# hallgeirl/cse168-raytracer

Measured on AMD Instinct MI355X. Metric: Mrays/s (primary+shadow), higher is better.
Workload: dtype f32; 1 GPU; sponza-standin 1920x1080 64spp primary+shadow; scene_triangles=76552, bvh_nodes=46701, math=exact: every quotient of the reference's slab and triangle tests, bit for bit, control_flow=while-while, ray_order=image order, resident_bytes_per_gpu=35765164

## Files before the change

### cse168-raytracer_amd/csrc/mr_api.cpp

```cpp
#include <algorithm>
#include <cmath>
#include <cstdarg>
#include <cstdio>
#include <cstring>
#include <new>
#include <vector>

#include "mr_internal.h"
#include "mr_tile.h"

namespace mr {

static thread_local char g_err[512] = "";

mr_status fail(mr_status code, const char *fmt, ...) {
    va_list ap;
    va_start(ap, fmt);
    vsnprintf(g_err, sizeof(g_err), fmt, ap);
    va_end(ap);
    return code;
}

namespace {

template <typename T>
mr_status upload(T *&dst, const T *src, size_t count, uint64_t &bytes) {
    const size_t sz = (count ? count : 1) * sizeof(T);
    MR_HIP_CHECK(hipMalloc(reinterpret_cast<void **>(&dst), sz));
    if (count) MR_HIP_CHECK(hipMemcpy(dst, src, count * sizeof(T), hipMemcpyHostToDevice));
    bytes += sz;
    return MR_OK;
}

void release_device(mr_scene *s) {
    DeviceScene &d = s->dev;
    (void)hipFree(d.nodes); (void)hipFree(d.tris); (void)hipFree(d.tri_prim); (void)hipFree(d.leaf_cnt_ext);
    (void)hipFree(d.v); (void)hipFree(d.n); (void)hipFree(d.vi); (void)hipFree(d.ni);
    (void)hipFree(d.materials); (void)hipFree(d.prim_material);
    (void)hipFree(d.spheres); (void)hipFree(d.planes);
    d = DeviceScene();
    (void)hipFree(s->d_stats); s->d_stats = nullptr;
    (void)hipFree(s->d_work_counters); s->d_work_counters = nullptr;
    for (EyeTables &t : s->eye_tables.set) {
        (void)hipFree(t.d);
        if (t.ready) (void)hipEventDestroy(static_cast<hipEvent_t>(t.ready));
        t = EyeTables();
    }
    s->eye_tables.calls = 0;
    (void)hipFree(s->d_stage_rays); (void)hipFree(s->d_stage_hits);
    s->d_stage_rays = s->d_stage_hits = nullptr;
    s->stage_cap = 0;
    for (void *e : s->stage_events) (void)hipEventDestroy(static_cast<hipEvent_t>(e));
    s->stage_events.clear();
    if (s->copy_in) (void)hipStreamDestroy(static_cast<hipStream_t>(s->copy_in));
    if (s->copy_out) (void)hipStreamDestroy(static_cast<hipStream_t>(s->copy_out));
    s->copy_in = s->copy_out = nullptr;
    (void)hipFree(s->d_occluded);
    s->d_occluded = nullptr;
    s->occluded_cap = 0;
    (void)hipFree(s->d_light_scale);
    s->d_light_scale = nullptr;
    s->light_scale_cap = 0;
}

inline int32_t leaf_ref(uint32_t first, uint32_t count) {
    const uint32_t c = count < (uint32_t)kLeafCountMask ? count : (uint32_t)kLeafCountMask;
    return (int32_t)~((first << kLeafCountBits) | c);
}

mr_status upload_materials(mr_scene *s);

std::vector<int32_t> node_storage_order(const HostTree &t, uint32_t mode) {
    std::vector<int32_t> order;
    const auto inner = [&](int32_t n) { return n >= 0 && !t.nodes[(size_t)n].is_leaf; };
    if (t.nodes.empty() || t.nodes[0].is_leaf) return order;
// ... 152 lines not shown
    if ((st = upload(d.tri_prim, rec_prim.data(), rec_prim.size(), d.bytes)) != MR_OK) return st;
    if ((st = upload(d.leaf_cnt_ext, cnt_ext.data(), cnt_ext.size(), d.bytes)) != MR_OK) return st;
    if ((st = upload(d.v, m.v.data(), m.v.size(), d.bytes)) != MR_OK) return st;
    if ((st = upload(d.n, m.n.data(), m.n.size(), d.bytes)) != MR_OK) return st;
    if ((st = upload(d.vi, m.vi.data(), m.vi.size(), d.bytes)) != MR_OK) return st;
    if ((st = upload(d.ni, m.ni.data(), m.ni.size(), d.bytes)) != MR_OK) return st;
    d.n_spheres = m.n_spheres();
    d.n_planes = m.n_planes();
    if (d.n_spheres) {
        std::vector<float4> sp(d.n_spheres);
        for (uint32_t i = 0; i < d.n_spheres; i++)
            sp[i] = make_float4(m.spheres[4 * i], m.spheres[4 * i + 1], m.spheres[4 * i + 2], m.spheres[4 * i + 3]);
        if ((st = upload(d.spheres, sp.data(), sp.size(), d.bytes)) != MR_OK) return st;
    }
    if (d.n_planes) {
        std::vector<float4> pl(2 * (size_t)d.n_planes);
        for (uint32_t i = 0; i < d.n_planes; i++) {
            float matf;
            memcpy(&matf, &m.plane_material[i], sizeof(matf));
            pl[2 * i] = make_float4(m.planes[6 * i], m.planes[6 * i + 1], m.planes[6 * i + 2], matf);
            pl[2 * i + 1] = make_float4(m.planes[6 * i + 3], m.planes[6 * i + 4], m.planes[6 * i + 5], 0.f);
        }
        if ((st = upload(d.planes, pl.data(), pl.size(), d.bytes)) != MR_OK) return st;
    }
    const HostNode &root = t.nodes[0];
    memcpy(d.root_lo, root.lo, sizeof(d.root_lo));
    memcpy(d.root_hi, root.hi, sizeof(d.root_hi));
    d.root_ref = ref_of(0);
    d.n_inner = n_inner;
    d.n_tris = n_rec;
    d.stack_depth = t.max_depth + 1;
    MR_HIP_CHECK(hipMalloc(reinterpret_cast<void **>(&s->d_stats), 2 * sizeof(unsigned long long)));
    MR_HIP_CHECK(hipMemset(s->d_stats, 0, 2 * sizeof(unsigned long long)));
    MR_HIP_CHECK(hipMalloc(reinterpret_cast<void **>(&s->d_work_counters), 2 * kWorkCounters * sizeof(unsigned long long)));
    MR_HIP_CHECK(hipMemset(s->d_work_counters, 0, 2 * kWorkCounters * sizeof(unsigned long long)));
    return upload_materials(s);
}

mr_status upload_materials(mr_scene *s) {
    DeviceScene &d = s->dev;
    if (!s->prim_material.empty() && s->prim_material.size() != s->mesh.n_triangles())
        return fail(MR_ERR_STATE, "mr_scene_set_materials covered %zu objects, the scene now holds %u: set the materials "
                                  "again after the last object was added", s->prim_material.size(), s->mesh.n_triangles());
    (void)hipFree(d.materials); (void)hipFree(d.prim_material);
    d.materials = nullptr; d.prim_material = nullptr;
    d.user_materials = s->materials.empty() ? 0u : 1u;
    d.refractive = 0;
    for (size_t i = 0; i + 10 < s->materials.size(); i += 11)
        if (s->materials[i + 6] > 0.f || s->materials[i + 7] > 0.f || s->materials[i + 8] > 0.f) d.refractive = 1;
    static const float white[11] = {1, 1, 1, 0, 0, 0, 0, 0, 0, 1, 1};
    const float *src = s->materials.empty() ? white : s->materials.data();
    const size_t nfl = s->materials.empty() ? 11 : s->materials.size();
    MR_HIP_CHECK(hipMalloc(reinterpret_cast<void **>(&d.materials), nfl * sizeof(float)));
    MR_HIP_CHECK(hipMemcpy(d.materials, src, nfl * sizeof(float), hipMemcpyHostToDevice));
    if (!s->prim_material.empty()) {
        MR_HIP_CHECK(hipMalloc(reinterpret_cast<void **>(&d.prim_material), s->prim_material.size() * sizeof(uint32_t)));
        MR_HIP_CHECK(hipMemcpy(d.prim_material, s->prim_material.data(), s->prim_material.size() * sizeof(uint32_t), hipMemcpyHostToDevice));
    }
    return MR_OK;
}

mr_status ensure_stage(mr_scene *s, uint64_t n) {
    if (n <= s->stage_cap) return MR_OK;
    (void)hipFree(s->d_stage_rays); (void)hipFree(s->d_stage_hits);
    s->d_stage_rays = s->d_stage_hits = nullptr;
    s->stage_cap = 0;
    MR_HIP_CHECK(hipMalloc(&s->d_stage_rays, n * sizeof(mr_ray)));
    MR_HIP_CHECK(hipMalloc(&s->d_stage_hits, n * sizeof(mr_hit)));
// ... 452 lines not shown
    for (uint32_t b = rank; b < nb; b += world) n += (b + 1) * band_rows <= H ? band_rows : H - b * band_rows;
    *rows = n;
    return MR_OK;
}

mr_status mr_deinterleave_bands(mr_scene *s, const float *d_recv, float *d_full, uint32_t W, uint32_t H, uint32_t band_rows,
                                uint32_t world, uint32_t shard_rows, uint32_t floats_per_pixel, void *stream) {
    mr_status st = require_device(s);
    if (st != MR_OK) return st;
    if (!d_recv || !d_full) return fail(MR_ERR_INVALID, "NULL argument");
    if (band_rows == 0 || world == 0 || floats_per_pixel == 0) return fail(MR_ERR_INVALID, "mr_deinterleave_bands: bad band description");
    for (uint32_t r = 0; r < world; r++) {
        uint32_t rows = 0;
        mr_band_rows_of(H, band_rows, r, world, &rows);
        if (rows > shard_rows) return fail(MR_ERR_INVALID, "rank %u owns %u rows, the shards hold %u", r, rows, shard_rows);
    }
    MR_HIP_CHECK(hipSetDevice(s->device));
    return launch_deinterleave(d_recv, d_full, W, H, band_rows, world, shard_rows, floats_per_pixel, static_cast<hipStream_t>(stream));
}

mr_status mr_render_direct(mr_scene *s, const mr_frame_desc *frame, float *d_rgb, mr_hit *d_hits, mr_hit *d_shadow_hits,
                           uint64_t *d_counts, void *stream) {
    mr_status st = require_device(s);
    if (st != MR_OK) return st;
    if (!frame || !d_rgb) return fail(MR_ERR_INVALID, "NULL argument");
    if (frame->W == 0 || frame->H == 0) return fail(MR_ERR_INVALID, "empty image");
    if ((reinterpret_cast<uintptr_t>(d_hits) & 15) || (reinterpret_cast<uintptr_t>(d_shadow_hits) & 15) ||
        (reinterpret_cast<uintptr_t>(d_counts) & 7) || (reinterpret_cast<uintptr_t>(d_rgb) & 3))
        return fail(MR_ERR_INVALID, "hit buffers must be 16-byte aligned, counters 8-byte aligned");
    mr_frame_desc fd = *frame;
    if (fd.band_world <= 1) { fd.band_world = 1; fd.band_rank = 0; if (fd.band_rows == 0) fd.band_rows = 1; }
    MR_HIP_CHECK(hipSetDevice(s->device));
    return launch_frame(s->dev, fd, d_rgb, d_hits, d_shadow_hits, reinterpret_cast<unsigned long long *>(d_counts),
                        s->d_work_counters + kWorkCounters + (s->next_counter.fetch_add(1) % kWorkCounters), s->eye_tables,
                        static_cast<hipStream_t>(stream));
}

mr_status mr_scene_set_materials(mr_scene *s, const mr_material *mats, uint32_t n_mats, const uint32_t *prim_material) {
    if (!s || !mats || n_mats == 0) return fail(MR_ERR_INVALID, "NULL argument or no materials");
    const uint32_t nt = s->mesh.n_triangles();
    if (prim_material)
        for (uint32_t i = 0; i < nt; i++)
            if (prim_material[i] >= n_mats) return fail(MR_ERR_INVALID, "triangle %u has material %u of %u", i, prim_material[i], n_mats);
    for (uint32_t i = 0; i < s->mesh.n_planes(); i++)
        if (s->mesh.plane_material[i] >= n_mats)
            return fail(MR_ERR_INVALID, "plane %u has material %u of %u", i, s->mesh.plane_material[i], n_mats);
    s->materials.resize(11 * (size_t)n_mats);
    for (uint32_t i = 0; i < n_mats; i++) {
        float *o = &s->materials[11 * (size_t)i];
        for (int c = 0; c < 3; c++) {
            const float ks = mats[i].specular[c];
            const float kt = fmaxf(fminf(mats[i].transmission[c], 1.0f - ks), 0.f);
            const float kd = fmaxf(fminf(mats[i].diffuse[c], 1.0f - ks - kt), 0.f);
            o[c] = kd; o[3 + c] = ks; o[6 + c] = kt;
        }
        o[9] = mats[i].shininess;
        o[10] = mats[i].refract_index;
    }
    if (prim_material) s->prim_material.assign(prim_material, prim_material + nt);
    else s->prim_material.clear();
    if (s->on_device) {
        MR_HIP_CHECK(hipSetDevice(s->device));
        MR_HIP_CHECK(hipDeviceSynchronize());
        return upload_materials(s);
    }
    return MR_OK;
}
// ... 161 lines not shown
```

### cse168-raytracer_amd/csrc/mr_frame.hip

```cpp
#include <hip/hip_runtime.h>

#include <cstring>

#include "mr_eye.h"
#include "mr_internal.h"
#include "mr_phong.h"
#include "mr_recursion.h"
#include "mr_surface.h"
#include "mr_tile.h"
#include "mr_traverse.h"

namespace mr {
namespace {

struct FrameArgs {
    EyeFrame eye;
    TraceParams tp;
    SurfacePtrs m;
    DirectLight lt;
    const float *mats;
    const uint32_t *prim_mat;
    mr_hit *hits;
    mr_hit *shadow_hits;
    float *rgb;
    unsigned long long *counts;
    uint32_t body_wgs, body_iters, tail_base, tail_chunks;
    unsigned *tail_counter;
    float4 *rel_nodes, *rel_tris;
    float rel_root_lo[3], rel_root_hi[3];
    uint32_t build, n_inner, n_rec;
};

__device__ __forceinline__ void eye_tables(const FrameArgs &a) {
    const unsigned i = blockIdx.x * (unsigned)kTraceBlock + threadIdx.x;
    const float ex = a.eye.eye[0], ey = a.eye.eye[1], ez = a.eye.eye[2];
    if (i < a.n_inner) {
        const float4 *q = a.tp.nodes + 4 * (size_t)i;
        const float4 q0 = q[0], q1 = q[1], q2 = q[2];
        int4 q3 = *reinterpret_cast<const int4 *>(q + 3);
        if (!(regular_pos(ex) && regular_pos(ey) && regular_pos(ez))) q3.z |= 1;
        float4 *d = a.rel_nodes + 4 * (size_t)i;
        d[0] = make_float4(q0.x - ex, q0.y - ex, q0.z - ey, q0.w - ey);
        d[1] = make_float4(q1.x - ex, q1.y - ex, q1.z - ey, q1.w - ey);
        d[2] = make_float4(q2.x - ez, q2.y - ez, q2.z - ez, q2.w - ez);
        *reinterpret_cast<int4 *>(d + 3) = q3;
    }
    if (i < a.n_rec) {
        const float4 *q = a.tp.tris + 3 * (size_t)i;
        const float4 q0 = q[0], q1 = q[1], q2 = q[2];
        const TriOriginTerms o = tri_origin_terms(q0, q1, q2, ex, ey, ez);
        float4 *d = a.rel_tris + 3 * (size_t)i;
        d[0] = make_float4(q2.y, q2.z, q2.w, o.pn);
        d[1] = make_float4(o.u.x, o.u.y, o.u.z, o.w.x);
        d[2] = make_float4(o.w.y, o.w.z, 0.0f, 0.0f);
    }
}

__device__ __forceinline__ unsigned tail_first_run(unsigned body_iters) {
    const unsigned q = body_iters >> 2;
    return q >= 8u ? 8u : q >= 4u ? 4u : q >= 2u ? 2u : 1u;
}
template <typename T>
__device__ __forceinline__ T kernarg_now(size_t offset) {
    typedef const volatile T __attribute__((address_space(4))) *ptr_t;
    const char __attribute__((address_space(4))) *ka = (const char __attribute__((address_space(4))) *)__builtin_amdgcn_kernarg_segment_ptr();
    return *(ptr_t)(ka + offset);
}

#ifndef MIRO_TAIL_PERMILLE
#define MIRO_TAIL_PERMILLE 60
#endif
#ifndef MIRO_BODY_ITERS
#define MIRO_BODY_ITERS 32
#endif
#ifndef MIRO_TAIL_MIN_CHUNKS
#define MIRO_TAIL_MIN_CHUNKS 60000ull
#endif
constexpr uint32_t kTailWgs = 1792 * (256 / kTraceBlock);
#ifndef MIRO_BODY_MIN_WGS
#define MIRO_BODY_MIN_WGS 14000
#endif
#ifndef MIRO_TAIL_PERMILLE_MID
#define MIRO_TAIL_PERMILLE_MID 60
#define MIRO_BODY_MIN_WGS_MID 14000
#endif
constexpr uint32_t kBodyMinWgs = MIRO_BODY_MIN_WGS;
struct FrameShape { uint32_t body_wgs, body_iters, tail_chunks, grid; };
inline FrameShape frame_schedule(unsigned long long chunks) {
    FrameShape s;
    if (chunks < MIRO_TAIL_MIN_CHUNKS || MIRO_TAIL_PERMILLE == 0 || kTraceBlock != 256) {
        const unsigned long long cap = chunks < kFrameLargeChunks ? (unsigned long long)kTraceGridCap : (unsigned long long)kFrameGridCapLarge;
        s.body_wgs = (uint32_t)(chunks < cap ? chunks : cap);
        s.body_iters = (uint32_t)((chunks + s.body_wgs - 1) / s.body_wgs);
        s.tail_chunks = 0;
        s.grid = s.body_wgs;
        return s;
    }
    const bool mid = chunks < kFrameLargeChunks;
    const unsigned long long tail_target = chunks * (mid ? MIRO_TAIL_PERMILLE_MID : MIRO_TAIL_PERMILLE) / 1000;
    uint32_t m = MIRO_BODY_ITERS;
    while (m > 1 && (chunks - tail_target) / m < (mid ? (uint32_t)MIRO_BODY_MIN_WGS_MID : kBodyMinWgs)) m >>= 1;
    while ((unsigned long long)m * (unsigned long long)kFrameGridCapLarge < chunks) m <<= 1;
    s.body_iters = m;
    s.body_wgs = (uint32_t)((chunks - tail_target) / m);
    s.tail_chunks = (uint32_t)(chunks - (unsigned long long)s.body_wgs * m);
    s.grid = s.body_wgs + kTailWgs;
    return s;
}

#if defined(MIRO_WG_TIMES) && MIRO_TRACE_BLOCK == 256
__device__ unsigned long long g_wg_times[4 * 131072];
#endif
template <int VAR, int SHADOW, bool MAT>
#ifndef MIRO_FRAME_WAVES
#define MIRO_FRAME_WAVES 7
#endif
__global__ __launch_bounds__(kTraceBlock) __attribute__((amdgpu_waves_per_eu(MIRO_FRAME_WAVES, 8))) void frame_kernel(FrameArgs a) {
#if defined(MIRO_WG_TIMES) && MIRO_TRACE_BLOCK == 256
    const unsigned long long wg_t0 = wall_clock64();
#endif
    constexpr bool kEyeRel = VAR == 794;
    if (kEyeRel && a.build) {
        eye_tables(a);
        return;
    }
    extern __shared__ int s_stack[];
    __shared__ unsigned s_shadow_rays[kTraceBlock / 64];
    const int tid = threadIdx.x;
    const unsigned long long n = a.eye.n, n_round = (n + 63ull) & ~63ull;
    constexpr bool kObj = (VAR & 32) != 0;
    const uint32_t spp = a.eye.spp;
    const float inv_spp = 1.0f / (float)spp;
    Stats st = {0ull, 0ull};
    unsigned my_shadow_rays = 0;

    __shared__ unsigned s_pull, s_run[2];
    if (tid == 0) { s_run[0] = 0; s_run[1] = 0; }
    unsigned long long idx, stride, limit;
    if (blockIdx.x < a.body_wgs) {
        const unsigned long long body_end = (unsigned long long)a.body_wgs * a.body_iters * kTraceBlock;
        idx = (unsigned long long)xcd_block_id_of(blockIdx.x, a.body_wgs, a.body_wgs >= (unsigned)kFrameGridCapLarge || a.tail_chunks != 0, a.tail_chunks != 0 ? 4096u : kXcdMinGrid) * kTraceBlock + tid;
        stride = (unsigned long long)a.body_wgs * kTraceBlock;
        limit = body_end < n_round ? body_end : n_round;
    } else {
        idx = 0; stride = 0; limit = n_round;
    }
    for (;; idx += stride) {
        if (__builtin_expect(stride == 0, 0)) {
            if (tid == 0) {
                unsigned left = s_run[1], next = s_run[0] + 1u;
                if (left == 0) {
                    const unsigned T = kernarg_now<uint32_t>(offsetof(FrameArgs, tail_chunks));
                    unsigned k = atomicAdd(kernarg_now<unsigned *>(offsetof(FrameArgs, tail_counter)), 1u);
                    s_pull = k;
                    unsigned at = 0;
                    next = 0xFFFFFFFFu;
                    for (unsigned size = tail_first_run(kernarg_now<uint32_t>(offsetof(FrameArgs, body_iters))); size >= 1; size >>= 1) {
                        const unsigned runs = size > 1 ? T / (4u * size) : T - at;
                        if (k < runs) { next = at + k * size; left = size; break; }
                        k -= runs;
                        at += runs * size;
                    }
                }
                s_run[0] = next;
                s_run[1] = next == 0xFFFFFFFFu ? 0u : left - 1u;
            }
            __syncthreads();
            const unsigned c = s_run[0];
            __syncthreads();
            if (c == 0xFFFFFFFFu) break;
            idx = ((unsigned long long)kernarg_now<uint32_t>(offsetof(FrameArgs, tail_base)) + c) * kTraceBlock + tid;
            if (idx >= limit) continue;
        } else if (idx >= limit) break;
        const bool live = idx < n;
        uint32_t x = 0, row = 0, y = 0, sm = 0;
        float4 ra = make_float4(0.f, 0.f, 0.f, 0.f), rb = make_float4(1.f, 1.f, 1.f, -1.f);
        if (live) {
            eye_sample_of(a.eye, idx, x, row, y, sm);
            eye_ray_of(a.eye, x, y, sm, ra, rb);
        }
        mr_hit h;
        {
            RayRegs r;
            ray_setup(r, ra, rb);
            Lane L;
            int plane_hit;
            if (kEyeRel) {
                TraceParams tp = a.tp;
                tp.nodes = a.rel_nodes; tp.tris = a.rel_tris;
                for (int k = 0; k < 3; k++) {
                    tp.root_lo[k] = kernarg_now<float>(offsetof(FrameArgs, rel_root_lo) + 4 * k);
                    tp.root_hi[k] = kernarg_now<float>(offsetof(FrameArgs, rel_root_hi) + 4 * k);
                }
                trace_ray<true, false, false, VAR, kEyeRel>(tp, r, rb.w, live, L, plane_hit, s_stack, tid, st);
            } else {
                trace_ray<true, false, false, VAR>(a.tp, r, rb.w, live, L, plane_hit, s_stack, tid, st);
            }
            h = make_hit<kObj>(a.tp, L, plane_hit, rb.w);
        }
        if (a.hits && live) reinterpret_cast<float4 *>(a.hits)[idx] = *reinterpret_cast<const float4 *>(&h);

        const bool hit = live && h.prim != MR_MISS;
        float c[3] = {0.f, 0.f, 0.f}, highlight = 0.0f;
        if (live && !hit) { c[0] = a.lt.bg[0]; c[1] = a.lt.bg[1]; c[2] = a.lt.bg[2]; }
// ... 21 lines not shown
            ray_setup(r, sa, sb);
            Lane L;
            int plane_hit;
            trace_ray<true, SHADOW == 1, false, VAR>(a.tp, r, sb.w, hit, L, plane_hit, s_stack, tid, st);
            mr_hit hs = make_hit<kObj>(a.tp, L, plane_hit, sb.w);
            if (!hit) { hs.t = 0.0f; hs.prim = MR_MISS; hs.beta = 0.0f; hs.gamma = 0.0f; }
            if (a.shadow_hits && live) reinterpret_cast<float4 *>(a.shadow_hits)[idx] = *reinterpret_cast<const float4 *>(&hs);
            if (MAT) {
                if (hit) {
                    rec::MeshMat mm;
                    mm.s = a.m; mm.mats = a.mats; mm.prim_mat = a.prim_mat;
                    rec::phong_combine(c, highlight, rec::light_scale_of(mm, sa, sb, *reinterpret_cast<const float4 *>(&hs)), c);
                }
            } else if (hs.prim != MR_MISS) {
                c[0] = 0.f; c[1] = 0.f; c[2] = 0.f;
            }
        } else {
            if (a.shadow_hits && live) reinterpret_cast<float4 *>(a.shadow_hits)[idx] = make_float4(0.0f, __uint_as_float(MR_MISS), 0.0f, 0.0f);
            if (MAT && hit) rec::phong_combine(c, highlight, 1.0f, c);
        }
        for (uint32_t off = 1; off < spp; off <<= 1) {
            c[0] += __shfl_xor(c[0], (int)off, 64);
            c[1] += __shfl_xor(c[1], (int)off, 64);
            c[2] += __shfl_xor(c[2], (int)off, 64);
        }
        if (live) eye_sample_of(a.eye, idx, x, row, y, sm);
        if (live && sm == 0) {
            if (spp > 1) { c[0] *= inv_spp; c[1] *= inv_spp; c[2] *= inv_spp; }
            float *o = a.rgb + 3 * ((size_t)row * a.eye.W + x);
            o[0] = c[0]; o[1] = c[1]; o[2] = c[2];
        }
    }

    if (stride == 0 && tid == 0) {
        const unsigned readers = gridDim.x - kernarg_now<uint32_t>(offsetof(FrameArgs, body_wgs));
        const unsigned T = kernarg_now<uint32_t>(offsetof(FrameArgs, tail_chunks));
        unsigned runs = 0, at = 0;
        for (unsigned size = tail_first_run(kernarg_now<uint32_t>(offsetof(FrameArgs, body_iters))); size >= 1; size >>= 1) {
            const unsigned r = size > 1 ? T / (4u * size) : T - at;
            runs += r;
            at += r * size;
        }
        if (s_pull == runs + readers - 1u) atomicExch(kernarg_now<unsigned *>(offsetof(FrameArgs, tail_counter)), 0u);
    }
    if (a.counts) {
        unsigned w = my_shadow_rays;
        for (int off = 32; off > 0; off >>= 1) w += __shfl_down(w, off, 64);
        if ((tid & 63) == 0) s_shadow_rays[tid >> 6] = w;
        __syncthreads();
        if (tid == 0) {
            unsigned long long tot = 0;
            for (int k = 0; k < kTraceBlock / 64; k++) tot += s_shadow_rays[k];
            if (tot) atomicAdd(&a.counts[1], tot);
            if (blockIdx.x == 0) atomicAdd(&a.counts[0], n);
        }
    }
#if defined(MIRO_WG_TIMES) && MIRO_TRACE_BLOCK == 256
    if (tid == 0 && blockIdx.x < 131072u) {
        g_wg_times[4 * blockIdx.x] = wg_t0;
        g_wg_times[4 * blockIdx.x + 1] = wall_clock64();
        g_wg_times[4 * blockIdx.x + 2] = __builtin_amdgcn_s_getreg((31 << 11) | 4);
        g_wg_times[4 * blockIdx.x + 3] = __builtin_amdgcn_s_getreg((31 << 11) | 20);
    }
#endif
}
#if defined(MIRO_WG_TIMES) && MIRO_TRACE_BLOCK == 256
}
}
extern "C" int mr_debug_wg_times(unsigned long long *out, unsigned n_words) {
    return (int)hipMemcpyFromSymbol(out, HIP_SYMBOL(mr::g_wg_times), (size_t)n_words * 8, 0, hipMemcpyDeviceToHost);
}
namespace mr {
namespace {
#endif

template <int VAR, int SHADOW, bool MAT>
mr_status launch_frame_t(FrameArgs a, hipStream_t stream) {
    const size_t lds = (size_t)a.tp.stack_depth * kTraceBlock * sizeof(int);
    if (lds > 150 * 1024) return fail(MR_ERR_INVALID, "traversal stack of depth %d does not fit in LDS", a.tp.stack_depth);
    if (lds > 48 * 1024)
        MR_HIP_CHECK(hipFuncSetAttribute(reinterpret_cast<const void *>(&frame_kernel<VAR, SHADOW, MAT>),
                                         hipFuncAttributeMaxDynamicSharedMemorySize, (int)lds));
    const FrameShape shape = frame_schedule((a.eye.n + kTraceBlock - 1) / kTraceBlock);
    a.body_wgs = shape.body_wgs; a.body_iters = shape.body_iters; a.tail_chunks = shape.tail_chunks;
    a.tail_base = shape.body_wgs * shape.body_iters;
    if (shape.tail_chunks && !a.tail_counter) return fail(MR_ERR_STATE, "mr_render_direct: no hand-out counter for the tail of a large frame");
    hipLaunchKernelGGL((frame_kernel<VAR, SHADOW, MAT>), dim3(shape.grid), dim3(kTraceBlock), lds, stream, a);
    MR_HIP_CHECK(hipGetLastError());
    return MR_OK;
}

template <int VAR>
mr_status launch_frame_plain(const FrameArgs &a, bool any, hipStream_t stream) {
    return any ? launch_frame_t<VAR, 1, false>(a, stream) : launch_frame_t<VAR, 0, false>(a, stream);
}
template <int VAR>
mr_status launch_frame_default(const FrameArgs &a, bool any, bool no_shadows, bool mat, hipStream_t stream) {
    if (mat) return no_shadows ? launch_frame_t<VAR, 2, true>(a, stream) : launch_frame_t<VAR, 0, true>(a, stream);
    if (no_shadows) return launch_frame_t<VAR, 2, false>(a, stream);
    return launch_frame_plain<VAR>(a, any, stream);
}

}

#ifndef MR_FRAME_ENTRY
#define MR_FRAME_ENTRY launch_frame_b256
#endif
static mr_status eye_tables_for(const DeviceScene &ds, EyeTablePool &pool, FrameArgs &a, hipStream_t stream) {
    hipStreamCaptureStatus cs = hipStreamCaptureStatusNone;
    MR_HIP_CHECK(hipStreamIsCapturing(stream, &cs));
    const bool capturing = cs != hipStreamCaptureStatusNone;
    std::lock_guard<std::mutex> lock(pool.mu);
    const uint64_t call = ++pool.calls;
    EyeTables *e = nullptr;
    if (!capturing)
        for (EyeTables &c : pool.set)
            if (c.reusable && memcmp(c.eye, a.eye.eye, sizeof(c.eye)) == 0) { e = &c; break; }
    const bool build = e == nullptr;
    if (build) {
// ... 6 lines not shown
            MR_HIP_CHECK(hipThreadExchangeStreamCaptureMode(&mode));
            hipError_t err = e->d ? hipSuccess : hipMalloc(reinterpret_cast<void **>(&e->d), eye_table_bytes(ds));
            if (err == hipSuccess && !e->ready)
                err = hipEventCreateWithFlags(reinterpret_cast<hipEvent_t *>(&e->ready), hipEventDisableTiming);
            MR_HIP_CHECK(hipThreadExchangeStreamCaptureMode(&mode));
            MR_HIP_CHECK(err);
        }
    } else if (e->stream != (void *)stream) {
        MR_HIP_CHECK(hipStreamWaitEvent(stream, static_cast<hipEvent_t>(e->ready), 0));
    }
    e->last_use = call;
    a.rel_nodes = e->d;
    a.rel_tris = e->d + 4 * (size_t)ds.n_inner;
    for (int c = 0; c < 3; c++) { a.rel_root_lo[c] = ds.root_lo[c] - a.eye.eye[c]; a.rel_root_hi[c] = ds.root_hi[c] - a.eye.eye[c]; }
    if (!build) return MR_OK;
    FrameArgs b = a;
    b.build = 1; b.n_inner = ds.n_inner; b.n_rec = ds.n_tris;
    const uint32_t n = ds.n_inner > ds.n_tris ? ds.n_inner : ds.n_tris;
    if (n) {
        hipLaunchKernelGGL((frame_kernel<794, 0, false>), dim3((n + kTraceBlock - 1) / kTraceBlock), dim3(kTraceBlock), 0, stream, b);
        MR_HIP_CHECK(hipGetLastError());
    }
    if (capturing) e->captured = true;
    if (!e->captured) {
        MR_HIP_CHECK(hipEventRecord(static_cast<hipEvent_t>(e->ready), stream));
        memcpy(e->eye, a.eye.eye, sizeof(e->eye));
        e->stream = (void *)stream;
        e->reusable = true;
    }
    return MR_OK;
}

mr_status MR_FRAME_ENTRY(const DeviceScene &ds, const mr_frame_desc &fd, float *d_rgb, mr_hit *d_hits, mr_hit *d_shadow_hits,
                         unsigned long long *d_counts, unsigned long long *work_counter, EyeTablePool &eye_pool, hipStream_t stream) {
    FrameArgs a;
    a.tail_counter = reinterpret_cast<unsigned *>(work_counter);
    a.rel_nodes = nullptr; a.rel_tris = nullptr;
    for (int c = 0; c < 3; c++) { a.rel_root_lo[c] = 0.0f; a.rel_root_hi[c] = 0.0f; }
    a.build = 0; a.n_inner = 0; a.n_rec = 0;
    const uint32_t spp = fd.spp;
    if (spp == 0 || spp > 64 || (spp & (spp - 1)))
        return fail(MR_ERR_INVALID, "mr_render_direct: spp must be a power of two <= 64 (got %u); use the batched pipeline", spp);
    if (fd.band_world == 0 || fd.band_rank >= fd.band_world || fd.band_rows == 0)
        return fail(MR_ERR_INVALID, "mr_render_direct: bad band description (%u rows, rank %u of %u)", fd.band_rows, fd.band_rank, fd.band_world);
    uint32_t rows = 0;
    if (fd.band_world == 1) {
        if (fd.y1 > fd.H || fd.y0 > fd.y1) return fail(MR_ERR_INVALID, "mr_render_direct: rows [%u,%u) outside the image", fd.y0, fd.y1);
        rows = fd.y1 - fd.y0;
    } else {
        const uint32_t nb = (fd.H + fd.band_rows - 1) / fd.band_rows;
        for (uint32_t b = fd.band_rank; b < nb; b += fd.band_world) {
            const uint32_t y0 = b * fd.band_rows, y1 = y0 + fd.band_rows < fd.H ? y0 + fd.band_rows : fd.H;
            rows += y1 - y0;
        }
    }
    a.eye = make_eye_frame(fd.camera, fd.W, fd.H, fd.band_world == 1 ? fd.y0 : 0, fd.band_world == 1 ? fd.y1 : rows, spp, fd.jitter, fd.seed,
                           fd.tiled != 0);
    a.eye.rows = rows;
    a.eye.n = (unsigned long long)rows * fd.W * spp;
    if (fd.band_world > 1) {
        a.eye.y0 = 0; a.eye.band_rows = fd.band_rows; a.eye.band_rank = fd.band_rank; a.eye.band_world = fd.band_world;
    }
    if (a.eye.n == 0) return MR_OK;
    if (a.eye.n >= (1ull << 32) * spp) return fail(MR_ERR_INVALID, "mr_render_direct: window too large");
    TraceParams &p = a.tp;
    p.nodes = ds.nodes; p.tris = ds.tris; p.tri_prim = ds.tri_prim; p.leaf_cnt_ext = ds.leaf_cnt_ext;
    for (int c = 0; c < 3; c++) { p.root_lo[c] = ds.root_lo[c]; p.root_hi[c] = ds.root_hi[c]; }
    p.root_ref = ds.root_ref;
    p.stack_depth = (int32_t)ds.stack_depth;
// ... 33 lines not shown
```

### cse168-raytracer_amd/csrc/mr_internal.h

```cpp
#pragma once

#include <hip/hip_runtime.h>

#include <atomic>
#include <mutex>
#include <cstdint>
#include <string>
#include <vector>

#include "miro_hip.h"

namespace mr {

mr_status fail(mr_status code, const char *fmt, ...);
#define MR_HIP_CHECK(expr)                                                              \
    do {                                                                                \
        hipError_t e__ = (expr);                                                        \
        if (e__ != hipSuccess)                                                          \
            return mr::fail(MR_ERR_HIP, "%s failed: %s (%s:%d)", #expr,                 \
                            hipGetErrorString(e__), __FILE__, __LINE__);                \
    } while (0)

struct HostNode {
    float lo[3], hi[3];
// ... 86 lines not shown
mr_status launch_shade(const DeviceScene &ds, const mr_ray *d_rays, const mr_hit *d_hits, unsigned long long n,
                       const mr_hit *d_shadow_hits, const uint32_t *d_shadow_src, const unsigned long long *d_shadow_count,
                       uint8_t *d_occluded, const mr_light &light, const float diffuse[3], uint32_t spp, float *d_rgb,
                       hipStream_t stream);
mr_status launch_gather_queries(const DeviceScene &ds, const mr_ray *d_rays, const mr_hit *d_hits, unsigned long long n,
                                float *d_pos, float *d_nrm, hipStream_t stream);
mr_status launch_gather_accumulate(const float *d_irr_a, const float *d_irr_b, unsigned long long n, uint32_t spp,
                                   float *d_rgb, hipStream_t stream);
mr_status launch_tonemap(const float *d_rgb, unsigned long long n_values, uint8_t *d_out, hipStream_t stream);
mr_status launch_deinterleave(const float *d_recv, float *d_full, uint32_t W, uint32_t H, uint32_t band_rows, uint32_t world,
                              uint32_t shard_rows, uint32_t fpp, hipStream_t stream);
mr_status launch_untile(const float *d_slots, float *d_image, uint32_t W, uint32_t rows, uint32_t spp, uint32_t channels,
                        hipStream_t stream);

struct EyeTables {
    float4 *d = nullptr;
    float eye[3] = {0.f, 0.f, 0.f};
    bool reusable = false;
    bool captured = false;
    uint64_t last_use = 0;
    void *ready = nullptr;
    void *stream = nullptr;
};
struct EyeTablePool {
    std::mutex mu;
    EyeTables set[kWorkCounters];
    uint64_t calls = 0;
};
inline size_t eye_table_bytes(const DeviceScene &ds) {
    const size_t b = (size_t)ds.n_inner * 64 + (size_t)ds.n_tris * 48;
    return b ? b : 64;
}
mr_status launch_frame_b256(const DeviceScene &ds, const mr_frame_desc &fd, float *d_rgb, mr_hit *d_hits, mr_hit *d_shadow_hits,
                            unsigned long long *d_counts, unsigned long long *work_counter, EyeTablePool &eye_pool, hipStream_t stream);
mr_status launch_frame_b128(const DeviceScene &ds, const mr_frame_desc &fd, float *d_rgb, mr_hit *d_hits, mr_hit *d_shadow_hits,
                            unsigned long long *d_counts, unsigned long long *work_counter, EyeTablePool &eye_pool, hipStream_t stream);
inline mr_status launch_frame(const DeviceScene &ds, const mr_frame_desc &fd, float *d_rgb, mr_hit *d_hits, mr_hit *d_shadow_hits,
                              unsigned long long *d_counts, unsigned long long *work_counter, EyeTablePool &eye_pool, hipStream_t stream) {
    const unsigned long long rows = fd.band_world > 1 ? (fd.H + fd.band_world - 1) / fd.band_world : (fd.y1 > fd.y0 ? fd.y1 - fd.y0 : 0);
    const unsigned long long samples = rows * fd.W * fd.spp;
    return samples <= 10000000ull ? launch_frame_b128(ds, fd, d_rgb, d_hits, d_shadow_hits, d_counts, work_counter, eye_pool, stream)
                                  : launch_frame_b256(ds, fd, d_rgb, d_hits, d_shadow_hits, d_counts, work_counter, eye_pool, stream);
}

mr_status launch_shade_accumulate(const DeviceScene &ds, const mr_ray *d_rays, const mr_hit *d_hits, const float *d_weights,
                                  const uint32_t *d_pixels, unsigned long long n, const mr_ray *d_shadow_rays,
                                  const mr_hit *d_shadow_hits, const uint32_t *d_shadow_src,
                                  const unsigned long long *d_shadow_count, float *d_light_scale, const mr_light &light,
                                  uint32_t spp, float *d_rgb, hipStream_t stream);
mr_status launch_secondary_rays(const DeviceScene &ds, const mr_ray *d_rays, const mr_hit *d_hits, const float *d_weights,
                                const uint32_t *d_pixels, unsigned long long n, uint32_t spp, mr_ray *d_out_rays,
                                float *d_out_weights, uint32_t *d_out_pixels, unsigned long long *d_count,
                                unsigned long long out_capacity, uint8_t *d_out_octants, hipStream_t stream);

mr_status launch_path_rays(const DeviceScene &ds, const mr_ray *d_rays, const mr_hit *d_hits, const float *d_weights,
                           const uint32_t *d_pixels, const uint32_t *d_ids, unsigned long long n, uint32_t spp, uint32_t seed,
                           uint32_t bounce, uint32_t kinds, mr_ray *d_out_rays, float *d_out_weights, uint32_t *d_out_pixels,
                           uint32_t *d_out_ids, unsigned long long *d_count, unsigned long long out_capacity, uint8_t *d_out_octants, hipStream_t stream);

mr_status launch_level(const DeviceScene &ds, const mr_level_desc &ld, const mr_ray *d_rays, const float *d_weights,
                       const uint32_t *d_pixels, const uint32_t *d_ids, unsigned long long n, float *d_rgb, mr_ray *d_out_rays,
                       float *d_out_weights, uint32_t *d_out_pixels, uint32_t *d_out_ids, unsigned long long *d_out_count,
                       unsigned long long *d_counts, hipStream_t stream);

struct ShadeLight {
    uint32_t kind;
    float position[3], normal[3], color[3], wattage, radius;
};
mr_status launch_shade_lights(const DeviceScene &ds, const ShadeLight *lights, uint32_t n_lights, const mr_ray *d_rays,
                              const mr_hit *d_hits, const float *d_weights, const uint32_t *d_pixels, unsigned long long n,
                              uint32_t spp, uint32_t flags, float *d_rgb, float *d_ray_rgb, unsigned long long *d_counts,
                              hipStream_t stream);

struct PhotonMapDev {
    float4 *rec = nullptr;
// ... 16 lines not shown
};
struct PhotonRoundHeader {
    uint32_t emitted;
    uint32_t reached;
    unsigned long long stored, segments;
};
struct PhotonRoundBuffers {
    float4 *slots = nullptr;
    float4 *compact = nullptr;
    uint32_t *words = nullptr;
    uint32_t *offsets = nullptr;
    unsigned *next = nullptr;
    PhotonRoundHeader *header = nullptr;
    uint32_t capacity = 0;
};
constexpr uint32_t kPhotonEventDomain = 0x70686f74u, kPhotonDiscDomain = 0x64697363u;
constexpr uint32_t kPhotonMaxDepth = 32;
mr_status launch_photon_round(const DeviceScene &ds, const PhotonWalkLight &lt, uint32_t seed, uint32_t caustic, uint32_t max_depth,
                              uint32_t first, uint32_t count, unsigned long long need, const PhotonRoundBuffers &b, hipStream_t stream);
int32_t photon_map_device(const mr_photon_map *m);
bool photon_map_balanced(const mr_photon_map *m);

}

struct mr_scene {
    int32_t device = 0;
    mr::HostMesh mesh;
    mr::HostTree tree;
    bool built = false;
    bool on_device = false;
    mr::DeviceScene dev;
    unsigned long long *d_stats = nullptr;
    unsigned long long *d_work_counters = nullptr;
    std::atomic<uint32_t> next_counter{0};
    mr::EyeTablePool eye_tables;
    void *d_stage_rays = nullptr, *d_stage_hits = nullptr;
    uint64_t stage_cap = 0;
    std::mutex stage_mutex;
    void *copy_in = nullptr, *copy_out = nullptr;
    std::vector<void *> stage_events;
    uint8_t *d_occluded = nullptr;
    uint64_t occluded_cap = 0;
    float *d_light_scale = nullptr;
    uint64_t light_scale_cap = 0;
    std::vector<float> materials;
    std::vector<uint32_t> prim_material;
    std::vector<mr::ShadeLight> lights;
};
```

Before: 17850 Mrays/s.

## Replace static body/tail split with per-XCD, per-CU dynamic chunk hand-out

```diff
diff --git a/cse168-raytracer_amd/csrc/mr_api.cpp b/cse168-raytracer_amd/csrc/mr_api.cpp
--- a/cse168-raytracer_amd/csrc/mr_api.cpp
+++ b/cse168-raytracer_amd/csrc/mr_api.cpp
@@ -6,6 +6,7 @@
 #include <new>
 #include <vector>
 
+#include "mr_handout.h"
 #include "mr_internal.h"
 #include "mr_tile.h"
 
@@ -41,6 +42,7 @@
     d = DeviceScene();
     (void)hipFree(s->d_stats); s->d_stats = nullptr;
     (void)hipFree(s->d_work_counters); s->d_work_counters = nullptr;
+    (void)hipFree(s->d_frame_handout); s->d_frame_handout = nullptr;
     for (EyeTables &t : s->eye_tables.set) {
         (void)hipFree(t.d);
         if (t.ready) (void)hipEventDestroy(static_cast<hipEvent_t>(t.ready));
@@ -259,8 +261,9 @@
     d.stack_depth = t.max_depth + 1;
     MR_HIP_CHECK(hipMalloc(reinterpret_cast<void **>(&s->d_stats), 2 * sizeof(unsigned long long)));
     MR_HIP_CHECK(hipMemset(s->d_stats, 0, 2 * sizeof(unsigned long long)));
-    MR_HIP_CHECK(hipMalloc(reinterpret_cast<void **>(&s->d_work_counters), 2 * kWorkCounters * sizeof(unsigned long long)));
-    MR_HIP_CHECK(hipMemset(s->d_work_counters, 0, 2 * kWorkCounters * sizeof(unsigned long long)));
+    MR_HIP_CHECK(hipMalloc(reinterpret_cast<void **>(&s->d_work_counters), kWorkCounters * sizeof(unsigned long long)));
+    MR_HIP_CHECK(hipMemset(s->d_work_counters, 0, kWorkCounters * sizeof(unsigned long long)));
+    MR_HIP_CHECK(hipMalloc(reinterpret_cast<void **>(&s->d_frame_handout), (size_t)kWorkCounters * kHoSlotBytes));
     return upload_materials(s);
 }
 
@@ -779,7 +782,7 @@
     if (fd.band_world <= 1) { fd.band_world = 1; fd.band_rank = 0; if (fd.band_rows == 0) fd.band_rows = 1; }
     MR_HIP_CHECK(hipSetDevice(s->device));
     return launch_frame(s->dev, fd, d_rgb, d_hits, d_shadow_hits, reinterpret_cast<unsigned long long *>(d_counts),
-                        s->d_work_counters + kWorkCounters + (s->next_counter.fetch_add(1) % kWorkCounters), s->eye_tables,
+                        s->d_frame_handout + (size_t)(s->next_counter.fetch_add(1) % kWorkCounters) * kHoSlotBytes, s->eye_tables,
                         static_cast<hipStream_t>(stream));
 }
 
diff --git a/cse168-raytracer_amd/csrc/mr_frame.hip b/cse168-raytracer_amd/csrc/mr_frame.hip
--- a/cse168-raytracer_amd/csrc/mr_frame.hip
+++ b/cse168-raytracer_amd/csrc/mr_frame.hip
@@ -1,8 +1,10 @@
 #include <hip/hip_runtime.h>
 
+#include <cstdlib>
 #include <cstring>
 
 #include "mr_eye.h"
+#include "mr_handout.h"
 #include "mr_internal.h"
 #include "mr_phong.h"
 #include "mr_recursion.h"
@@ -24,11 +26,12 @@
     mr_hit *shadow_hits;
     float *rgb;
     unsigned long long *counts;
-    uint32_t body_wgs, body_iters, tail_base, tail_chunks;
-    unsigned *tail_counter;
+    uint32_t body_wgs, body_iters, ho_key_shift, ho_unused;
+    unsigned char *ho_slot;
     float4 *rel_nodes, *rel_tris;
     float rel_root_lo[3], rel_root_hi[3];
     uint32_t build, n_inner, n_rec;
+    HandoutShape ho;
 };
 
 __device__ __forceinline__ void eye_tables(const FrameArgs &a) {
@@ -56,10 +59,6 @@
     }
 }
 
-__device__ __forceinline__ unsigned tail_first_run(unsigned body_iters) {
-    const unsigned q = body_iters >> 2;
-    return q >= 8u ? 8u : q >= 4u ? 4u : q >= 2u ? 2u : 1u;
-}
 template <typename T>
 __device__ __forceinline__ T kernarg_now(size_t offset) {
     typedef const volatile T __attribute__((address_space(4))) *ptr_t;
@@ -70,43 +69,51 @@
 #ifndef MIRO_TAIL_PERMILLE
 #define MIRO_TAIL_PERMILLE 60
 #endif
-#ifndef MIRO_BODY_ITERS
-#define MIRO_BODY_ITERS 32
-#endif
-#ifndef MIRO_TAIL_MIN_CHUNKS
-#define MIRO_TAIL_MIN_CHUNKS 60000ull
-#endif
-constexpr uint32_t kTailWgs = 1792 * (256 / kTraceBlock);
-#ifndef MIRO_BODY_MIN_WGS
-#define MIRO_BODY_MIN_WGS 14000
-#endif
-#ifndef MIRO_TAIL_PERMILLE_MID
-#define MIRO_TAIL_PERMILLE_MID 60
-#define MIRO_BODY_MIN_WGS_MID 14000
-#endif
-constexpr uint32_t kBodyMinWgs = MIRO_BODY_MIN_WGS;
-struct FrameShape { uint32_t body_wgs, body_iters, tail_chunks, grid; };
-inline FrameShape frame_schedule(unsigned long long chunks) {
+#ifndef MIRO_HANDOUT_MIN_CHUNKS
+#define MIRO_HANDOUT_MIN_CHUNKS 60000ull
+#endif
+#ifndef MIRO_HANDOUT_RUN
+#define MIRO_HANDOUT_RUN 16
+#define MIRO_HANDOUT_PULL 2
+#define MIRO_HANDOUT_KEY_SHIFT 0
+#endif
+constexpr uint32_t kFrameSlots = 1792;
+struct FrameShape { uint32_t body_wgs, body_iters, grid; bool handout; };
+inline FrameShape frame_schedule(unsigned long long chunks, unsigned long long handout_min = MIRO_HANDOUT_MIN_CHUNKS) {
     FrameShape s;
-    if (chunks < MIRO_TAIL_MIN_CHUNKS || MIRO_TAIL_PERMILLE == 0 || kTraceBlock != 256) {
-        const unsigned long long cap = chunks < kFrameLargeChunks ? (unsigned long long)kTraceGridCap : (unsigned long long)kFrameGridCapLarge;
-        s.body_wgs = (uint32_t)(chunks < cap ? chunks : cap);
-        s.body_iters = (uint32_t)((chunks + s.body_wgs - 1) / s.body_wgs);
-        s.tail_chunks = 0;
-        s.grid = s.body_wgs;
+    s.handout = chunks >= handout_min && kTraceBlock == 256;
+    if (s.handout) {
+        s.body_wgs = 0; s.body_iters = 0; s.grid = kFrameSlots;
         return s;
     }
-    const bool mid = chunks < kFrameLargeChunks;
-    const unsigned long long tail_target = chunks * (mid ? MIRO_TAIL_PERMILLE_MID : MIRO_TAIL_PERMILLE) / 1000;
-    uint32_t m = MIRO_BODY_ITERS;
-    while (m > 1 && (chunks - tail_target) / m < (mid ? (uint32_t)MIRO_BODY_MIN_WGS_MID : kBodyMinWgs)) m >>= 1;
-    while ((unsigned long long)m * (unsigned long long)kFrameGridCapLarge < chunks) m <<= 1;
-    s.body_iters = m;
-    s.body_wgs = (uint32_t)((chunks - tail_target) / m);
-    s.tail_chunks = (uint32_t)(chunks - (unsigned long long)s.body_wgs * m);
-    s.grid = s.body_wgs + kTailWgs;
+    const unsigned long long cap = chunks < kFrameLargeChunks ? (unsigned long long)kTraceGridCap : (unsigned long long)kFrameGridCapLarge;
+    s.body_wgs = (uint32_t)(chunks < cap ? chunks : cap);
+    s.body_iters = (uint32_t)((chunks + s.body_wgs - 1) / s.body_wgs);
+    s.grid = s.body_wgs;
     return s;
 }
+struct HandoutShapeNow {
+    static __device__ __forceinline__ uint32_t field(size_t offset);
+    __device__ uint32_t run() const { return field(offsetof(HandoutShape, run_)); }
+    __device__ uint32_t pull() const { return field(offsetof(HandoutShape, pull_)); }
+    __device__ uint32_t xcd_runs() const { return field(offsetof(HandoutShape, xcd_runs_)); }
+    __device__ uint32_t body_chunks() const { return field(offsetof(HandoutShape, body_chunks_)); }
+    __device__ uint32_t tail_chunks() const { return field(offsetof(HandoutShape, tail_chunks_)); }
+    __device__ uint32_t tail_first() const { return field(offsetof(HandoutShape, tail_first_)); }
+};
+__device__ __forceinline__ uint32_t HandoutShapeNow::field(size_t offset) { return kernarg_now<uint32_t>(offsetof(FrameArgs, ho) + offset); }
+struct HandoutSlot {
+    unsigned char *base;
+    __device__ uint64_t cursor_add(uint32_t i, uint32_t n) {
+        return atomicAdd(reinterpret_cast<unsigned long long *>(base + (size_t)i * kHoCursorBytes), (unsigned long long)n);
+    }
+    __device__ bool cursor_cas(uint32_t i, uint64_t expected, uint64_t desired) {
+        return atomicCAS(reinterpret_cast<unsigned long long *>(base + (size_t)i * kHoCursorBytes), (unsigned long long)expected,
+                         (unsigned long long)desired) == expected;
+    }
+    __device__ uint32_t xcd_add(uint32_t x) { return atomicAdd(reinterpret_cast<unsigned *>(base + kHoXcdOffset + x * kHoCounterBytes), 1u); }
+    __device__ uint32_t tail_add() { return atomicAdd(reinterpret_cast<unsigned *>(base + kHoTailOffset), 1u); }
+};
 
 #if defined(MIRO_WG_TIMES) && MIRO_TRACE_BLOCK == 256
 __device__ unsigned long long g_wg_times[4 * 131072];
@@ -121,7 +128,12 @@
 #endif
     constexpr bool kEyeRel = VAR == 794;
     if (kEyeRel && a.build) {
-        eye_tables(a);
+        if (a.build == 2) {
+            const unsigned i = blockIdx.x * (unsigned)kTraceBlock + threadIdx.x;
+            if (i < kHoSlotBytes / 4u) reinterpret_cast<uint32_t *>(a.ho_slot)[i] = 0u;
+        } else {
+            eye_tables(a);
+        }
         return;
     }
     extern __shared__ int s_stack[];
@@ -134,12 +146,13 @@
     Stats st = {0ull, 0ull};
     unsigned my_shadow_rays = 0;
 
-    __shared__ unsigned s_pull, s_run[2];
-    if (tid == 0) { s_run[0] = 0; s_run[1] = 0; }
+    __shared__ HandoutLocal s_ho;
+    __shared__ unsigned s_chunk;
+    if (tid == 0) handout_local_init(s_ho);
     unsigned long long idx, stride, limit;
     if (blockIdx.x < a.body_wgs) {
         const unsigned long long body_end = (unsigned long long)a.body_wgs * a.body_iters * kTraceBlock;
-        idx = (unsigned long long)xcd_block_id_of(blockIdx.x, a.body_wgs, a.body_wgs >= (unsigned)kFrameGridCapLarge || a.tail_chunks != 0, a.tail_chunks != 0 ? 4096u : kXcdMinGrid) * kTraceBlock + tid;
+        idx = (unsigned long long)xcd_block_id_of(blockIdx.x, a.body_wgs, a.body_wgs >= (unsigned)kFrameGridCapLarge) * kTraceBlock + tid;
         stride = (unsigned long long)a.body_wgs * kTraceBlock;
         limit = body_end < n_round ? body_end : n_round;
     } else {
@@ -148,28 +161,23 @@
     for (;; idx += stride) {
         if (__builtin_expect(stride == 0, 0)) {
             if (tid == 0) {
-                unsigned left = s_run[1], next = s_run[0] + 1u;
-                if (left == 0) {
-                    const unsigned T = kernarg_now<uint32_t>(offsetof(FrameArgs, tail_chunks));
-                    unsigned k = atomicAdd(kernarg_now<unsigned *>(offsetof(FrameArgs, tail_counter)), 1u);
-                    s_pull = k;
-                    unsigned at = 0;
-                    next = 0xFFFFFFFFu;
-                    for (unsigned size = tail_first_run(kernarg_now<uint32_t>(offsetof(FrameArgs, body_iters))); size >= 1; size >>= 1) {
-                        const unsigned runs = size > 1 ? T / (4u * size) : T - at;
-                        if (k < runs) { next = at + k * size; left = size; break; }
-                        k -= runs;
-                        at += runs * size;
-                    }
+                HandoutLocal l = s_ho;
+                if (l.left == 0) {
+                    HandoutShapeNow hs;
+                    HandoutSlot slot = {kernarg_now<unsigned char *>(offsetof(FrameArgs, ho_slot))};
+                    const unsigned xcd = __builtin_amdgcn_s_getreg((31 << 11) | 20) & 0xFu, cu = (__builtin_amdgcn_s_getreg((31 << 11) | 4) >> 8) & 0xFFu;
+                    handout_pull(slot, hs, xcd, cu >> kernarg_now<uint32_t>(offsetof(FrameArgs, ho_key_shift)), l);
                 }
-                s_run[0] = next;
-                s_run[1] = next == 0xFFFFFFFFu ? 0u : left - 1u;
+                unsigned c = kHoNone;
+                if (l.left != 0) { c = l.next; l.next++; l.left--; }
+                s_ho = l;
+                s_chunk = c;
             }
             __syncthreads();
-            const unsigned c = s_run[0];
+            const unsigned c = s_chunk;
             __syncthreads();
-            if (c == 0xFFFFFFFFu) break;
-            idx = ((unsigned long long)kernarg_now<uint32_t>(offsetof(FrameArgs, tail_base)) + c) * kTraceBlock + tid;
+            if (c == kHoNone) break;
+            idx = (unsigned long long)c * kTraceBlock + tid;
             if (idx >= limit) continue;
         } else if (idx >= limit) break;
         const bool live = idx < n;
@@ -257,17 +265,6 @@
         }
     }
 
-    if (stride == 0 && tid == 0) {
-        const unsigned readers = gridDim.x - kernarg_now<uint32_t>(offsetof(FrameArgs, body_wgs));
-        const unsigned T = kernarg_now<uint32_t>(offsetof(FrameArgs, tail_chunks));
-        unsigned runs = 0, at = 0;
-        for (unsigned size = tail_first_run(kernarg_now<uint32_t>(offsetof(FrameArgs, body_iters))); size >= 1; size >>= 1) {
-            const unsigned r = size > 1 ? T / (4u * size) : T - at;
-            runs += r;
-            at += r * size;
-        }
-        if (s_pull == runs + readers - 1u) atomicExch(kernarg_now<unsigned *>(offsetof(FrameArgs, tail_counter)), 0u);
-    }
     if (a.counts) {
         unsigned w = my_shadow_rays;
         for (int off = 32; off > 0; off >>= 1) w += __shfl_down(w, off, 64);
@@ -306,10 +303,28 @@
     if (lds > 48 * 1024)
         MR_HIP_CHECK(hipFuncSetAttribute(reinterpret_cast<const void *>(&frame_kernel<VAR, SHADOW, MAT>),
                                          hipFuncAttributeMaxDynamicSharedMemorySize, (int)lds));
-    const FrameShape shape = frame_schedule((a.eye.n + kTraceBlock - 1) / kTraceBlock);
-    a.body_wgs = shape.body_wgs; a.body_iters = shape.body_iters; a.tail_chunks = shape.tail_chunks;
-    a.tail_base = shape.body_wgs * shape.body_iters;
-    if (shape.tail_chunks && !a.tail_counter) return fail(MR_ERR_STATE, "mr_render_direct: no hand-out counter for the tail of a large frame");
+    const unsigned long long chunks = (a.eye.n + kTraceBlock - 1) / kTraceBlock;
+    uint32_t run = MIRO_HANDOUT_RUN, pull = MIRO_HANDOUT_PULL;
+    unsigned long long handout_min = MIRO_HANDOUT_MIN_CHUNKS;
+    a.ho_key_shift = MIRO_HANDOUT_KEY_SHIFT; a.ho_unused = 0;
+#ifdef MIRO_DEV
+    if (const char *e = getenv("MIRO_HANDOUT_RUN")) run = (uint32_t)atoi(e);
+    if (const char *e = getenv("MIRO_HANDOUT_PULL")) pull = (uint32_t)atoi(e);
+    if (const char *e = getenv("MIRO_HANDOUT_KEY_SHIFT")) a.ho_key_shift = (uint32_t)atoi(e);
+    if (const char *e = getenv("MIRO_HANDOUT_MIN_CHUNKS")) handout_min = strtoull(e, nullptr, 10);
+    if (run == 0 || run > kHoStripe || (run & (run - 1)) || pull == 0 || pull > run || (pull & (pull - 1)) || a.ho_key_shift > 7)
+        return fail(MR_ERR_INVALID, "bad hand-out parameters in the environment");
+#endif
+    const FrameShape shape = frame_schedule(chunks, handout_min);
+    a.body_wgs = shape.body_wgs; a.body_iters = shape.body_iters;
+    a.ho = handout_shape(chunks, run, pull, MIRO_TAIL_PERMILLE);
+    if (shape.handout) {
+        if (!a.ho_slot) return fail(MR_ERR_STATE, "mr_render_direct: no hand-out counters for a large frame");
+        FrameArgs b = a;
+        b.build = 2;
+        hipLaunchKernelGGL((frame_kernel<794, 0, false>), dim3((kHoSlotBytes / 4u + kTraceBlock - 1) / kTraceBlock), dim3(kTraceBlock), 0, stream, b);
+        MR_HIP_CHECK(hipGetLastError());
+    }
     hipLaunchKernelGGL((frame_kernel<VAR, SHADOW, MAT>), dim3(shape.grid), dim3(kTraceBlock), lds, stream, a);
     MR_HIP_CHECK(hipGetLastError());
     return MR_OK;
@@ -382,9 +397,9 @@
 }
 
 mr_status MR_FRAME_ENTRY(const DeviceScene &ds, const mr_frame_desc &fd, float *d_rgb, mr_hit *d_hits, mr_hit *d_shadow_hits,
-                         unsigned long long *d_counts, unsigned long long *work_counter, EyeTablePool &eye_pool, hipStream_t stream) {
+                         unsigned long long *d_counts, unsigned char *handout_slot, EyeTablePool &eye_pool, hipStream_t stream) {
     FrameArgs a;
-    a.tail_counter = reinterpret_cast<unsigned *>(work_counter);
+    a.ho_slot = handout_slot;
     a.rel_nodes = nullptr; a.rel_tris = nullptr;
     for (int c = 0; c < 3; c++) { a.rel_root_lo[c] = 0.0f; a.rel_root_hi[c] = 0.0f; }
     a.build = 0; a.n_inner = 0; a.n_rec = 0;
diff --git a/cse168-raytracer_amd/csrc/mr_handout.h b/cse168-raytracer_amd/csrc/mr_handout.h
--- /dev/null
+++ b/cse168-raytracer_amd/csrc/mr_handout.h
@@ -0,0 +1,105 @@
+#pragma once
+
+#include <stdint.h>
+
+#if defined(__HIPCC__)
+#define MR_HO_FN __host__ __device__ inline
+#else
+#define MR_HO_FN inline
+#endif
+#if defined(__clang__)
+#define MR_HO_NOUNROLL _Pragma("nounroll")
+#else
+#define MR_HO_NOUNROLL
+#endif
+
+namespace mr {
+
+constexpr uint32_t kHoNone = 0xFFFFFFFFu;
+constexpr uint32_t kHoStripe = 256;
+constexpr uint32_t kHoXcds = 8;
+constexpr uint32_t kHoCuIds = 128;
+constexpr uint32_t kHoCursors = kHoXcds * kHoCuIds;
+constexpr uint32_t kHoCursorBytes = 64, kHoCounterBytes = 128;
+constexpr uint32_t kHoXcdOffset = kHoCursors * kHoCursorBytes;
+constexpr uint32_t kHoTailOffset = kHoXcdOffset + kHoXcds * kHoCounterBytes;
+constexpr uint32_t kHoSlotBytes = kHoTailOffset + kHoCounterBytes;
+
+struct HandoutShape {
+    uint32_t run_, pull_, xcd_runs_, body_chunks_, tail_chunks_, tail_first_;
+    MR_HO_FN uint32_t run() const { return run_; }
+    MR_HO_FN uint32_t pull() const { return pull_; }
+    MR_HO_FN uint32_t xcd_runs() const { return xcd_runs_; }
+    MR_HO_FN uint32_t body_chunks() const { return body_chunks_; }
+    MR_HO_FN uint32_t tail_chunks() const { return tail_chunks_; }
+    MR_HO_FN uint32_t tail_first() const { return tail_first_; }
+};
+
+MR_HO_FN HandoutShape handout_shape(unsigned long long chunks, uint32_t run, uint32_t pull, uint32_t tail_permille) {
+    HandoutShape s;
+    s.run_ = run; s.pull_ = pull;
+    const unsigned long long group = (unsigned long long)kHoXcds * kHoStripe;
+    const unsigned long long groups = (chunks - chunks * tail_permille / 1000) / group;
+    s.body_chunks_ = (uint32_t)(groups * group);
+    s.xcd_runs_ = (uint32_t)(groups * (kHoStripe / run));
+    s.tail_chunks_ = (uint32_t)(chunks - groups * group);
+    s.tail_first_ = run < 8u ? run : 8u;
+    return s;
+}
+
+template <class SHAPE>
+MR_HO_FN uint32_t handout_body_run(const SHAPE &s, uint32_t x, uint32_t v) {
+    if (v >= s.xcd_runs()) return kHoNone;
+    const uint32_t per = kHoStripe >> __builtin_ctz(s.run()), g = v >> __builtin_ctz(per), w = v & (per - 1u);
+    return (g * kHoXcds + x) * kHoStripe + w * s.run();
+}
+
+template <class SHAPE>
+MR_HO_FN uint32_t handout_tail_run(const SHAPE &s, uint32_t k, uint32_t &len) {
+    uint32_t at = 0;
+    for (uint32_t size = s.tail_first(); size >= 1; size >>= 1) {
+        const uint32_t runs = size > 1 ? s.tail_chunks() >> (2 + __builtin_ctz(size)) : s.tail_chunks() - at;
+        if (k < runs) { len = size; return s.body_chunks() + at + k * size; }
+        k -= runs;
+        at += runs * size;
+    }
+    len = 0;
+    return kHoNone;
+}
+
+struct HandoutLocal {
+    uint32_t next, left;
+    uint32_t backlog;
+    uint32_t tail_only;
+};
+MR_HO_FN void handout_local_init(HandoutLocal &l) { l.next = 0; l.left = 0; l.backlog = kHoNone; l.tail_only = 0; }
+
+template <class MEM, class SHAPE>
+MR_HO_FN void handout_pull(MEM &mem, const SHAPE &s, uint32_t xcd_id, uint32_t cu_id, HandoutLocal &l) {
+    const uint32_t x = xcd_id % kHoXcds, cursor = x * kHoCuIds + cu_id % kHoCuIds;
+MR_HO_NOUNROLL
+    for (int attempt = 0; attempt < 2 && !l.tail_only; attempt++) {
+        const uint64_t w = mem.cursor_add(cursor, s.pull());
+        const uint32_t first1 = (uint32_t)(w >> 32), off = (uint32_t)w;
+        if (first1 != 0 && off < s.run()) {
+            l.next = first1 - 1u + off;
+            l.left = s.run() - off < s.pull() ? s.run() - off : s.pull();
+            return;
+        }
+MR_HO_NOUNROLL
+        for (uint32_t i = 0; i < kHoXcds && l.backlog == kHoNone; i++)
+            l.backlog = handout_body_run(s, (x + i) % kHoXcds, mem.xcd_add((x + i) % kHoXcds));
+        if (l.backlog == kHoNone) { l.tail_only = 1; break; }
+        if (mem.cursor_cas(cursor, w + s.pull(), ((uint64_t)(l.backlog + 1u) << 32) | s.pull())) {
+            l.next = l.backlog; l.left = s.pull(); l.backlog = kHoNone;
+            return;
+        }
+    }
+    if (l.backlog != kHoNone) {
+        l.next = l.backlog; l.left = s.run(); l.backlog = kHoNone;
+        return;
+    }
+    l.next = handout_tail_run(s, mem.tail_add(), l.left);
+}
+
+}
diff --git a/cse168-raytracer_amd/csrc/mr_internal.h b/cse168-raytracer_amd/csrc/mr_internal.h
--- a/cse168-raytracer_amd/csrc/mr_internal.h
+++ b/cse168-raytracer_amd/csrc/mr_internal.h
@@ -142,15 +142,15 @@
     return b ? b : 64;
 }
 mr_status launch_frame_b256(const DeviceScene &ds, const mr_frame_desc &fd, float *d_rgb, mr_hit *d_hits, mr_hit *d_shadow_hits,
-                            unsigned long long *d_counts, unsigned long long *work_counter, EyeTablePool &eye_pool, hipStream_t stream);
+                            unsigned long long *d_counts, unsigned char *handout_slot, EyeTablePool &eye_pool, hipStream_t stream);
 mr_status launch_frame_b128(const DeviceScene &ds, const mr_frame_desc &fd, float *d_rgb, mr_hit *d_hits, mr_hit *d_shadow_hits,
-                            unsigned long long *d_counts, unsigned long long *work_counter, EyeTablePool &eye_pool, hipStream_t stream);
+                            unsigned long long *d_counts, unsigned char *handout_slot, EyeTablePool &eye_pool, hipStream_t stream);
 inline mr_status launch_frame(const DeviceScene &ds, const mr_frame_desc &fd, float *d_rgb, mr_hit *d_hits, mr_hit *d_shadow_hits,
-                              unsigned long long *d_counts, unsigned long long *work_counter, EyeTablePool &eye_pool, hipStream_t stream) {
+                              unsigned long long *d_counts, unsigned char *handout_slot, EyeTablePool &eye_pool, hipStream_t stream) {
     const unsigned long long rows = fd.band_world > 1 ? (fd.H + fd.band_world - 1) / fd.band_world : (fd.y1 > fd.y0 ? fd.y1 - fd.y0 : 0);
     const unsigned long long samples = rows * fd.W * fd.spp;
-    return samples <= 10000000ull ? launch_frame_b128(ds, fd, d_rgb, d_hits, d_shadow_hits, d_counts, work_counter, eye_pool, stream)
-                                  : launch_frame_b256(ds, fd, d_rgb, d_hits, d_shadow_hits, d_counts, work_counter, eye_pool, stream);
+    return samples <= 10000000ull ? launch_frame_b128(ds, fd, d_rgb, d_hits, d_shadow_hits, d_counts, handout_slot, eye_pool, stream)
+                                  : launch_frame_b256(ds, fd, d_rgb, d_hits, d_shadow_hits, d_counts, handout_slot, eye_pool, stream);
 }
 
 mr_status launch_shade_accumulate(const DeviceScene &ds, const mr_ray *d_rays, const mr_hit *d_hits, const float *d_weights,
@@ -233,6 +233,7 @@
     mr::DeviceScene dev;
     unsigned long long *d_stats = nullptr;
     unsigned long long *d_work_counters = nullptr;
+    unsigned char *d_frame_handout = nullptr;
     std::atomic<uint32_t> next_counter{0};
     mr::EyeTablePool eye_tables;
     void *d_stage_rays = nullptr, *d_stage_hits = nullptr;
```

Result: slower. 16890 Mrays/s (-5.4%).
